# dmlc/dgl

Hardware: AMD Instinct MI355X
Metric: edges/sec for g-SpMM copy_u+sum (feat=100); % HBM roofline (higher is better)
Workload: dtype f32; 1 GPU; configs[1]: g-SpMM copy_u+sum on ogbn-products-shaped CSR (N=2449029 rows, E=61859140 edges, feat=100) fp32, int32 ids, variant U; parallelism=1 GPU, tuning_flags=25

## Files before the change

dgl_amd/csrc/spmm_csr.hip.h:

```cpp
#pragma once
#include <algorithm>
#include <cstdlib>
#include <type_traits>

#include "common.h"

namespace dgla {

template <typename Idx>
struct SpmmParams {
  const Idx* indptr;
  const Idx* indices;
  const Idx* eids;
  int64_t num_rows, nnz, num_waves;
  int wave_items;
  const int64_t* plan;
  const void* ufeat;
  const void* efeat;
  void* out;
  Idx* arg_u;
  Idx* arg_e;
  int out_len, lhs_len, rhs_len;
  int log2_lpe;
  int rhs_group;
  BcastDims bd;
  int accumulate;
  int rhs_neg, rhs_div;
  int rhs_mask;
  int stage_w;
  int red_min;
  int arg_empty;
  int mean;
  uint32_t tune;
  const void* umain;
  const void* utail;
  const unsigned* split_meta;
  int split_main, split_tail;
  int split_edge_lines;
  int split_t16;
  int split_base16;
  int split_straddle_slack;
  int split_row_bytes, split_base_bytes;
  const uint8_t* rel;
  const void* const* xtab;
  const void* const* wtab;
  int num_rel;
  int wave_slots;
  unsigned* fix_count;
  int64_t* carry_row;
  void* carry_val;
  void* tail_val;
  Idx* carry_argu;
  Idx* carry_arge;
  Idx* tail_argu;
  Idx* tail_arge;
};

template <typename Idx>
__global__ void spmm_merge_plan_kernel(const Idx* __restrict__ indptr, int64_t num_rows,
                                       int64_t nnz, int64_t num_waves,
                                       int64_t* __restrict__ plan, int wave_items) {
  const int64_t w = blockIdx.x * static_cast<int64_t>(blockDim.x) + threadIdx.x;
  if (w > num_waves) return;
  int64_t d = w * wave_items;
  const int64_t total = num_rows + nnz;
  if (d > total) d = total;
  int64_t lo = 0, hi = num_rows;
  while (lo < hi) {
    const int64_t mid = (lo + hi + 1) >> 1;
    if (static_cast<int64_t>(indptr[mid]) + mid <= d)
      lo = mid;
    else
      hi = mid - 1;
  }
  plan[w] = lo;
}

template <typename DT, int VEC>
__device__ __forceinline__ void store_nt(DT* dst, const VecT<DT, VEC>& v) {
  constexpr int B = sizeof(DT) * VEC;
  if constexpr (B == 16) {
// ... 168 lines not shown
}
template <typename T>
__device__ __forceinline__ void st_sc1(T* p, T v) {
  __hip_atomic_store((__attribute__((address_space(1))) T*)p, v, __ATOMIC_RELAXED, __HIP_MEMORY_SCOPE_AGENT);
}

template <typename DT>
__device__ __forceinline__ bool mask_bit(DT w, int k) {
  if constexpr (sizeof(DT) == 2) {
    uint16_t b;
    __builtin_memcpy(&b, &w, 2);
    return (b >> (k & 15)) & 1;
  } else if constexpr (sizeof(DT) == 4) {
    uint32_t b;
    __builtin_memcpy(&b, &w, 4);
    return (b >> (k & 31)) & 1;
  } else {
    uint64_t b;
    __builtin_memcpy(&b, &w, 8);
    return (b >> (k & 63)) & 1;
  }
}

template <typename Idx, typename DT, int VEC, int OP, int RED, int BC, int U, bool MULTI = false,
          bool NTR = false>
__global__ __launch_bounds__(64 * kWavesPerBlock) void spmm_csr_merge_kernel(
    const SpmmParams<Idx> p) {
  using A = typename Acc<DT>::type;
  constexpr bool UL = op_uses_lhs(OP), UR = op_uses_rhs(OP);
  constexpr bool ARG = RED != kSum;
  constexpr bool TU = UL && !MULTI, TE = UR || MULTI;
  constexpr int RV = (BC == kBcNone) ? VEC : 1;

  __shared__ int s_cols[UL ? kWavesPerBlock : 1][UL ? kWaveItems : 1];
  __shared__ int s_rend[kWavesPerBlock][kWaveItems + 2];
  extern __shared__ __align__(8) unsigned char s_dyn[];
  __shared__ uint8_t s_rel[MULTI ? kWavesPerBlock : 1][MULTI ? kWaveItems : 1];
  __shared__ const DT* s_tx[(MULTI && UL) ? 256 : 1];
  __shared__ const DT* s_tw[(MULTI && UR) ? 256 : 1];
  if constexpr (MULTI) {
    for (int i = threadIdx.x; i < p.num_rel; i += 64 * kWavesPerBlock) {
      if constexpr (UL) s_tx[i] = static_cast<const DT*>(p.xtab[i]);
      if constexpr (UR) s_tw[i] = static_cast<const DT*>(p.wtab[i]);
    }
  }

  const int wib = threadIdx.x >> 6;
  const int lane = threadIdx.x & 63;
  unsigned blk = blockIdx.x;
  if ((p.tune & kTuneXcd) && gridDim.y == 1) {
    const unsigned nb = gridDim.x, q = nb >> 3, r = nb & 7u;
    const unsigned x = blk & 7u, i = blk >> 3;
    blk = x * q + (x < r ? x : r) + i;
  }
  const int64_t w = static_cast<int64_t>(blk) * kWavesPerBlock + wib;
  const bool has_eid = p.eids != nullptr;
  constexpr bool kStageW = UL && UR && !MULTI && !NTR && BC == kBcRhsGroup && RED == kSum && sizeof(DT) == 4;
  [[maybe_unused]] const bool stage_w = kStageW && p.stage_w != 0;

  int64_t i0 = 0, j0 = 0;
  int R = 0, nE = 0;
  if (w < p.num_waves) {
    const int64_t total = p.num_rows + p.nnz;
    const int64_t d0 = w * p.wave_items;
    int64_t d1 = d0 + p.wave_items;
    if (d1 > total) d1 = total;
    i0 = p.plan[w];
    const int64_t i1 = p.plan[w + 1];
    j0 = d0 - i0;
    R = static_cast<int>(i1 - i0);
    nE = static_cast<int>((d1 - i1) - j0);
    const int items = nE + R;
    if (items > 0) {
      Idx itemv[kWaveItems / 64];
      Idx eidv[kWaveItems / 64];
      [[maybe_unused]] uint32_t wv[kStageW ? kWaveItems / 64 : 1];
      uint8_t relv[MULTI ? kWaveItems / 64 : 1];
#pragma unroll
      for (int k = 0; k < kWaveItems / 64; ++k) {
        if (64 * k >= p.wave_items) break;
        int it = lane + 64 * k;
        if (it >= items) it = items - 1;
        const Idx* src = p.indptr + (i0 + 1 + (it < nE ? 0 : it - nE));
        if constexpr (UL) src = it < nE ? p.indices + (j0 + it) : src;
        itemv[k] = *src;
        if constexpr (MULTI) relv[k] = it < nE ? p.rel[j0 + it] : uint8_t(0);
        if constexpr (UR) {
          if (has_eid) {
            const int ie = it < nE ? it : (nE > 0 ? nE - 1 : 0);
            eidv[k] = nE > 0 ? load_global<Idx, 1>(p.eids + (j0 + ie)).v[0] : static_cast<Idx>(p.arg_empty);
          }
          if constexpr (kStageW) {
            if (stage_w && !has_eid)
              wv[k] = nE > 0 ? load_global<uint32_t, 1>(static_cast<const uint32_t*>(p.efeat) + (j0 + (it < nE ? it : nE - 1))).v[0] : 0u;
          }
        }
      }
      if constexpr (kStageW) {
        if (stage_w && has_eid) {
#pragma unroll
          for (int k = 0; k < kWaveItems / 64; ++k) {
            if (64 * k >= p.wave_items) break;
            wv[k] = nE > 0 ? load_global<uint32_t, 1>(static_cast<const uint32_t*>(p.efeat) + static_cast<int64_t>(eidv[k])).v[0] : 0u;
          }
        }
      }
      const int64_t first = static_cast<int64_t>(p.indptr[i0]) - j0;
#pragma unroll
      for (int k = 0; k < kWaveItems / 64; ++k) {
        if (64 * k >= p.wave_items) break;
        const int it = lane + 64 * k;
        if (it < nE) {
          if constexpr (UL) s_cols[wib][it] = static_cast<int>(itemv[k]);
          if constexpr (UR) {
            bool staged = false;
            if constexpr (kStageW) {
              if (stage_w) {
                reinterpret_cast<uint32_t*>(s_dyn)[wib * kWaveItems + it] = wv[k];
                staged = true;
              }
            }
            if (!staged && has_eid) reinterpret_cast<Idx*>(s_dyn)[wib * kWaveItems + it] = eidv[k];
          }
          if constexpr (MULTI) s_rel[wib][it] = relv[k];
        } else if (it < items) {
          s_rend[wib][it - nE + 1] = static_cast<int>(static_cast<int64_t>(itemv[k]) - j0);
        }
      }
      if (lane == 0) s_rend[wib][0] = first < 0 ? -1 : static_cast<int>(first);
    } else if (lane == 0) {
      s_rend[wib][0] = 0;
    }
  }
  __syncthreads();
  if (w >= p.num_waves) return;

  const int lpe = 1 << p.log2_lpe;
  const int g = lane >> p.log2_lpe;
  const int lg = lane & (lpe - 1);
  const int G = 64 >> p.log2_lpe;
  const int Tg = p.wave_items >> (6 - p.log2_lpe);
  const int F = p.out_len;
  const int k0 = (static_cast<int>(blockIdx.y) * 64 + lg) * VEC;
  if (k0 >= F) return;

  typedef const __attribute__((address_space(3))) int* lds_int_ptr;
  typedef const __attribute__((address_space(3))) Idx* lds_idx_ptr;
  const lds_int_ptr cols = (lds_int_ptr)s_cols[UL ? wib : 0];
  const lds_int_ptr rend = (lds_int_ptr)s_rend[wib];
  const lds_idx_ptr eidl = (lds_idx_ptr)s_dyn + wib * kWaveItems;

  const int items = R + nE;
  int dlo = g * Tg, dhi = dlo + Tg;
  if (dlo > items) dlo = items;
  if (dhi > items) dhi = items;
  auto rows_before = [&](int d) {
    int lo = 0, hi = R;
    while (lo < hi) {
      const int mid = (lo + hi) >> 1;
      if (rend[mid + 1] + mid < d)
        lo = mid + 1;
      else
        hi = mid;
    }
    return lo;
  };
  const int t_s = rows_before(dlo), t_e = rows_before(dhi);
  const int e_s = dlo - t_s, e_e = dhi - t_e;
  const bool wslots = (RED == kSum) && p.wave_slots != 0;
  const int64_t slot = wslots ? w : w * G + g;

  int lo_off = k0, ro_off = k0;
  if constexpr (BC == kBcRhsGroup) ro_off = k0 / p.rhs_group;
  if constexpr (BC == kBcGeneral) bcast_offsets(p.bd, k0, &lo_off, &ro_off);
  const DT* __restrict__ X = static_cast<const DT*>(p.ufeat) + lo_off;
  const DT* __restrict__ Wt = static_cast<const DT*>(p.efeat) + ro_off;
  const int64_t lhs_len = p.lhs_len;
  const int64_t rhs_len = p.rhs_len;
  constexpr int E16 = 16 / static_cast<int>(sizeof(DT));
  bool edge_layout = false;
  [[maybe_unused]] unsigned ej = 0u;
  [[maybe_unused]] int e_piece_lo = 0, e_piece_hi = 0;
  [[maybe_unused]] int e_pitch = 0;
  [[maybe_unused]] const DT* e_side = nullptr;
  bool straddle = false;
  if (p.split_main > 0 && p.split_straddle_slack >= 0) {
    if constexpr (UL && !MULTI && VEC * sizeof(DT) == 8) straddle = split_wanted(p.split_meta);
  } else if (p.split_main > 0 && p.split_edge_lines > 0 && split_wanted(p.split_meta)) {
    {
      if constexpr (UL && !MULTI && VEC * sizeof(DT) == 16) {
        edge_layout = true;
        const int j = lo_off / E16, rp = p.lhs_len / E16;
        if (j >= rp - p.split_t16) {
          ej = 0x40000000u;
          e_side = static_cast<const DT*>(p.utail);
          e_pitch = p.split_t16 * E16;
          e_piece_lo = e_piece_hi = (j - (rp - p.split_t16)) * E16;
        } else {
          ej = static_cast<unsigned>(j);
          e_side = static_cast<const DT*>(p.umain);
          e_pitch = 8 * E16;
// ... 96 lines not shown
            const unsigned head = 8u - o16;
            const bool in_place = (ej - head) < e_in_place;
            const int side_off = ej < head ? e_piece_lo : e_piece_hi;
            const DT* base = in_place ? X : e_side;
            const int64_t pitch = in_place ? lhs_len : static_cast<int64_t>(e_pitch);
            const int add = in_place ? 0 : side_off;
            ptr = reinterpret_cast<const XV*>(base + (c * pitch + add));
            done = true;
          }
        }
        if constexpr (VEC * sizeof(DT) == 8) {
          if (straddle) {
            const unsigned o = static_cast<unsigned>((static_cast<uint64_t>(c) * static_cast<unsigned>(p.split_row_bytes) +
                                                      static_cast<unsigned>(p.split_base_bytes)) & 127u);
            const bool from_side = o > static_cast<unsigned>(p.split_straddle_slack);
            const DT* base = from_side ? static_cast<const DT*>(p.umain) + lo_off : X;
            const int64_t pitch = from_side ? static_cast<int64_t>(p.split_main) : lhs_len;
            ptr = reinterpret_cast<const XV*>(base + c * pitch);
            done = true;
          }
        }
        if (!done) ptr = reinterpret_cast<const XV*>(X + c * lhs_len);
        uint64_t wb = 0;
        __builtin_memcpy(&wb, &b.w[u].v[0], sizeof(DT));
        const bool wanted = ((wb >> (k0 & (BITS - 1))) & ((1u << VEC) - 1u)) != 0u;
        b.x[u] = *(wanted ? ptr : gate_dummy);
      }
    }
  };

  [[maybe_unused]] auto load_batch_sw = [&](int e, Batch& b) {
    if constexpr (kStageW) {
      typedef const __attribute__((address_space(3))) uint32_t* lds_u32_ptr;
      const lds_u32_ptr sw = (lds_u32_ptr)s_dyn + wib * kWaveItems;
#pragma unroll
      for (int u = 0; u < U; ++u) {
        int ee = e + u;
        if (ee >= e_e) ee = e_e - 1;
        const int64_t c = cols[ee];
        bool done = false;
        if constexpr (VEC * sizeof(DT) == 16) {
          if (edge_layout) {
            const unsigned o16 = (e_t16 * static_cast<unsigned>(c) + e_base16) & 7u;
            const unsigned head = 8u - o16;
            const bool in_place = (ej - head) < e_in_place;
            const int side_off = ej < head ? e_piece_lo : e_piece_hi;
            const DT* base = in_place ? X : e_side;
            const int64_t pitch = in_place ? lhs_len : static_cast<int64_t>(e_pitch);
            const int add = in_place ? 0 : side_off;
            b.x[u] = *reinterpret_cast<const XV*>(base + (c * pitch + add));
            done = true;
          }
        }
        if constexpr (VEC * sizeof(DT) == 8) {
          if (straddle) {
            const unsigned o = static_cast<unsigned>((static_cast<uint64_t>(c) * static_cast<unsigned>(p.split_row_bytes) +
                                                      static_cast<unsigned>(p.split_base_bytes)) & 127u);
            const bool from_side = o > static_cast<unsigned>(p.split_straddle_slack);
            const DT* base = from_side ? static_cast<const DT*>(p.umain) + lo_off : X;
            const int64_t pitch = from_side ? static_cast<int64_t>(p.split_main) : lhs_len;
            b.x[u] = *reinterpret_cast<const XV*>(base + c * pitch);
            done = true;
          }
        }
        if (!done) b.x[u] = *reinterpret_cast<const XV*>(X + c * lhs_len);
        const uint32_t wbits = sw[ee];
        __builtin_memcpy(&b.w[u].v[0], &wbits, 4);
// ... 19 lines not shown
  auto edge_name = [&](int bi) -> Idx {
    if (bi < 0) return static_cast<Idx>(p.arg_empty);
    if constexpr (MULTI)
      return static_cast<Idx>(j0 + bi);
    else if constexpr (UR)
      return has_eid ? eidl[bi] : static_cast<Idx>(j0 + bi);
    else
      return Idx(0);
  };
  DT* __restrict__ out = static_cast<DT*>(p.out);
  bool first_is_tail = rend[t_s] < e_s;
  [[maybe_unused]] A treg[VEC];
  [[maybe_unused]] bool have_tail = false;
  [[maybe_unused]] int tail_t = 0;

  const bool fuse = p.fix_count != nullptr;
  [[maybe_unused]] int64_t tail_pending = -1;
  auto put_part = [&](A* dst, const A (&vals)[VEC]) {
    if (fuse) {
#pragma unroll
      for (int v = 0; v < VEC; ++v) st_sc1(dst + v, vals[v]);
    } else {
#pragma unroll
      for (int v = 0; v < VEC; ++v) dst[v] = vals[v];
    }
  };
  auto put_arg = [&](Idx* dst, Idx val) {
    if (fuse)
      st_sc1(dst, val);
    else
      *dst = val;
  };

  auto flush = [&](int t) {
    const int64_t row = i0 + t;
    if (first_is_tail && RED == kSum && wslots && g == 1) {
#pragma unroll
      for (int v = 0; v < VEC; ++v) treg[v] = acc[v];
      have_tail = true;
      tail_t = t;
      first_is_tail = false;
    } else if (first_is_tail) {
      put_part(static_cast<A*>(p.tail_val) + slot * F + k0, acc);
      if constexpr (ARG) {
#pragma unroll
        for (int v = 0; v < VEC; ++v) {
          const int bi = best[v];
          if constexpr (TU) put_arg(p.tail_argu + slot * F + k0 + v, bi >= 0 ? static_cast<Idx>(cols[bi]) : static_cast<Idx>(p.arg_empty));
          if constexpr (TE) put_arg(p.tail_arge + slot * F + k0 + v, edge_name(bi));
        }
      }
      tail_pending = row;
      first_is_tail = false;
    } else {
      DT* o = out + row * F + k0;
      VecT<DT, VEC> ov;
      if (p.accumulate) {
        ov = *reinterpret_cast<VecT<DT, VEC>*>(o);
#pragma unroll
        for (int v = 0; v < VEC; ++v) ov.v[v] = from_acc<DT>(to_acc<DT>(ov.v[v]) + acc[v]);
      } else if (RED == kSum && p.mean) {
        const A den = round_to_storage<DT>(static_cast<A>(cnt > 1 ? cnt : 1));
#pragma unroll
        for (int v = 0; v < VEC; ++v) ov.v[v] = from_acc<DT>(round_to_storage<DT>(acc[v]) / den);
      } else {
#pragma unroll
        for (int v = 0; v < VEC; ++v) ov.v[v] = from_acc<DT>(acc[v]);
      }
// ... 55 lines not shown
            if constexpr (TE) ae[v] = geti(pe + base + v);
          }
        }
      }
    };
    for (int64_t q = s_first + 1; q < s_last; ++q) combine(cv, p.carry_argu, p.carry_arge, q * F + k0);
    combine(tv, p.tail_argu, p.tail_arge, s_last * F + k0);
    DT* o = out + R * F + k0;
    VecT<DT, VEC> ov;
    if (RED == kSum && p.mean) {
      const int64_t deg = rb - ra;
      const A den = round_to_storage<DT>(static_cast<A>(deg > 1 ? deg : 1));
#pragma unroll
      for (int v = 0; v < VEC; ++v) ov.v[v] = from_acc<DT>(round_to_storage<DT>(tot[v]) / den);
    } else if (p.accumulate) {
      ov = *reinterpret_cast<VecT<DT, VEC>*>(o);
#pragma unroll
      for (int v = 0; v < VEC; ++v) ov.v[v] = from_acc<DT>(to_acc<DT>(ov.v[v]) + tot[v]);
    } else {
#pragma unroll
      for (int v = 0; v < VEC; ++v) ov.v[v] = from_acc<DT>(tot[v]);
    }
    *reinterpret_cast<VecT<DT, VEC>*>(o) = ov;
    if constexpr (ARG) {
#pragma unroll
      for (int v = 0; v < VEC; ++v) {
        if constexpr (TU) p.arg_u[R * F + k0 + v] = au[v];
        if constexpr (TE) p.arg_e[R * F + k0 + v] = ae[v];
      }
    }
  };

  int t = t_s;
  int next_end = (t < R) ? rend[t + 1] : 0x7fffffff;
  [[maybe_unused]] const bool rhs_neg = p.rhs_neg != 0, rhs_div = p.rhs_div != 0, rhs_mask = p.rhs_mask != 0;

  auto reduce_batch = [&](int e, const Batch& b) {
#pragma unroll
    for (int u = 0; u < U; ++u) {
      const int ee = e + u;
      if (ee < e_e) {
        while (ee >= next_end) {
          flush(t);
          ++t;
          next_end = (t < R) ? rend[t + 1] : 0x7fffffff;
        }
#pragma unroll
        for (int v = 0; v < VEC; ++v) {
          A l = A(0), r = A(0);
          if constexpr (UL) l = to_acc<DT>(b.x[u].v[v]);
          if constexpr (UR) r = to_acc<DT>(b.w[u].v[RV == 1 ? 0 : v]);
          A raw;
          if constexpr (OP == kAdd)
            raw = l + (rhs_neg ? -r : r);
          else if constexpr (OP == kMul && BC == kBcRhsGroup)
            raw = rhs_mask ? (mask_bit<DT>(b.w[u].v[0], k0 + v) ? l : A(0)) : (rhs_div ? l / r : l * r);
          else if constexpr (OP == kMul)
            raw = rhs_div ? l / r : l * r;
          else
            raw = apply_op<OP, A>(l, r);
          const A val = round_to_storage<DT>(raw);
          if constexpr (RED == kSum) {
            acc[v] += val;
          } else {
            if (red_min ? acc[v] > val : acc[v] < val) {
              acc[v] = val;
              best[v] = ee;
            }
          }
        }
        ++cnt;
      }
    }
  };

  bool gated_done = false;
  if constexpr (kGated) {
    if (rhs_mask && VEC <= static_cast<int>(8 * sizeof(DT)) && (p.tune & kTuneNoGate) == 0) {
// ... 19 lines not shown
    }
  }
  if constexpr (kStageW) {
    if (stage_w && !gated_done) {
      gated_done = true;
      if (e_s < e_e) {
        int e = e_s;
        Batch ba, bb;
        load_batch_sw(e, ba);
        for (; e < e_e; e += 2 * U) {
          load_batch_sw(e + U, bb);
          reduce_batch(e, ba);
          load_batch_sw(e + 2 * U, ba);
          reduce_batch(e + U, bb);
        }
      }
    }
  }
  if (!gated_done && e_s < e_e) {
    int e = e_s;
    Batch ba, bb;
    load_batch(e, ba);
    for (; e < e_e; e += 2 * U) {
      load_batch(e + U, bb);
      reduce_batch(e, ba);
      load_batch(e + 2 * U, ba);
      reduce_batch(e + U, bb);
    }
  }
  while (t < t_e) {
    flush(t);
    ++t;
  }

  if constexpr (RED == kSum) {
    if (wslots) {
      A c0[VEC];
#pragma unroll
      for (int v = 0; v < VEC; ++v) c0[v] = __shfl_xor(acc[v], 32, 64);
      const int cnt0 = __shfl_xor(cnt, 32, 64);
      if (g == 1) {
        const bool g0_carry = cnt0 > 0;
        int64_t crow = -1;
        if (have_tail) {
          A tot[VEC];
#pragma unroll
          for (int v = 0; v < VEC; ++v) tot[v] = c0[v] + treg[v];
          const bool began_here = tail_t > 0 || rend[0] >= 0;
          if (began_here) {
            DT* o = out + (i0 + tail_t) * F + k0;
            VecT<DT, VEC> ov;
            if (p.accumulate) {
              ov = *reinterpret_cast<VecT<DT, VEC>*>(o);
#pragma unroll
              for (int v = 0; v < VEC; ++v) ov.v[v] = from_acc<DT>(to_acc<DT>(ov.v[v]) + tot[v]);
            } else if (p.mean) {
              const int deg = rend[tail_t + 1] - rend[tail_t];
              const A den = round_to_storage<DT>(static_cast<A>(deg > 1 ? deg : 1));
#pragma unroll
              for (int v = 0; v < VEC; ++v) ov.v[v] = from_acc<DT>(round_to_storage<DT>(tot[v]) / den);
            } else {
#pragma unroll
              for (int v = 0; v < VEC; ++v) ov.v[v] = from_acc<DT>(tot[v]);
            }
            *reinterpret_cast<VecT<DT, VEC>*>(o) = ov;
          } else {
            put_part(static_cast<A*>(p.tail_val) + slot * F + k0, tot);
            tail_pending = i0 + tail_t;
          }
          if (cnt > 0) {
            crow = i0 + t;
            put_part(static_cast<A*>(p.carry_val) + slot * F + k0, acc);
          }
        } else if (g0_carry || cnt > 0) {
          crow = i0 + t;
          A cvv[VEC];
#pragma unroll
          for (int v = 0; v < VEC; ++v) cvv[v] = g0_carry ? (cnt > 0 ? c0[v] + acc[v] : c0[v]) : acc[v];
          put_part(static_cast<A*>(p.carry_val) + slot * F + k0, cvv);
        }
        if (!fuse && lg == 0) p.carry_row[slot] = crow;
        if (fuse && crow >= 0) finish_run(crow);
      }
      if (fuse && tail_pending >= 0) finish_run(tail_pending);
      return;
    }
  }
  const bool has_carry = cnt > 0;
  if (!fuse && lg == 0 && blockIdx.y == 0) p.carry_row[slot] = has_carry ? i0 + t : int64_t(-1);
  if (has_carry) {
    put_part(static_cast<A*>(p.carry_val) + slot * F + k0, acc);
    if constexpr (ARG) {
#pragma unroll
      for (int v = 0; v < VEC; ++v) {
        const int bi = best[v];
        if constexpr (TU) put_arg(p.carry_argu + slot * F + k0 + v, bi >= 0 ? static_cast<Idx>(cols[bi]) : static_cast<Idx>(p.arg_empty));
        if constexpr (TE) put_arg(p.carry_arge + slot * F + k0 + v, edge_name(bi));
      }
    }
  }
  if (fuse) {
    if (tail_pending >= 0) finish_run(tail_pending);
    if (has_carry) finish_run(i0 + t);
  }
}

template <typename Idx, typename DT, int OP, int RED, bool MULTI = false>
__global__ __launch_bounds__(64) void spmm_csr_fixup_kernel(const SpmmParams<Idx> p,
                                                            int64_t num_slots) {
  using A = typename Acc<DT>::type;
  constexpr bool UL = op_uses_lhs(OP) && !MULTI, UR = op_uses_rhs(OP) || MULTI;
  constexpr bool ARG = RED != kSum;
  for (int64_t s = blockIdx.x; s < num_slots; s += gridDim.x) {
    const int64_t row = p.carry_row[s];
    if (row < 0) continue;
    if (s > 0 && p.carry_row[s - 1] == row) continue;
    int64_t s2 = s + 1;
    for (;;) {
      const int64_t q = s2 + threadIdx.x;
      const bool same = q < num_slots && p.carry_row[q] == row;
      const uint64_t m = __ballot(same);
      if (m != ~uint64_t(0)) {
        s2 += __builtin_ctzll(~m);
        break;
      }
      s2 += 64;
    }
    const int F = p.out_len;
    const A* cv = static_cast<const A*>(p.carry_val);
    const A* tv = static_cast<const A*>(p.tail_val);
    DT* out = static_cast<DT*>(p.out);
    for (int k = threadIdx.x; k < F; k += 64) {
      A acc = cv[s * F + k];
      Idx au = 0, ae = 0;
      if constexpr (ARG) {
        if constexpr (UL) au = p.carry_argu[s * F + k];
        if constexpr (UR) ae = p.carry_arge[s * F + k];
      }
      auto combine = [&](A val, Idx cu, Idx ce) {
        if constexpr (RED == kSum) {
          acc += val;
        } else {
          const bool take = p.red_min ? (acc > val) : (acc < val);
          if (take) {
            acc = val;
            if constexpr (UL) au = cu;
            if constexpr (UR) ae = ce;
          }
        }
      };
      const A tval = tv[s2 * F + k];
      Idx tu = 0, te = 0;
      if constexpr (ARG) {
        if constexpr (UL) tu = p.tail_argu[s2 * F + k];
        if constexpr (UR) te = p.tail_arge[s2 * F + k];
      }
      int64_t q = s + 1;
      for (; q + 8 <= s2; q += 8) {
        A v[8];
        Idx vu[8], ve[8];
#pragma unroll
        for (int u = 0; u < 8; ++u) {
          v[u] = cv[(q + u) * F + k];
          vu[u] = ve[u] = 0;
          if constexpr (ARG) {
            if constexpr (UL) vu[u] = p.carry_argu[(q + u) * F + k];
            if constexpr (UR) ve[u] = p.carry_arge[(q + u) * F + k];
          }
        }
#pragma unroll
        for (int u = 0; u < 8; ++u) combine(v[u], vu[u], ve[u]);
      }
      for (; q < s2; ++q) {
        Idx cu = 0, ce = 0;
        if constexpr (ARG) {
          if constexpr (UL) cu = p.carry_argu[q * F + k];
          if constexpr (UR) ce = p.carry_arge[q * F + k];
        }
        combine(cv[q * F + k], cu, ce);
      }
      combine(tval, tu, te);
      const int64_t o = row * F + k;
      if (RED == kSum && p.mean) {
        const int64_t deg = static_cast<int64_t>(p.indptr[row + 1]) - static_cast<int64_t>(p.indptr[row]);
        acc = round_to_storage<DT>(acc) / round_to_storage<DT>(static_cast<A>(deg > 1 ? deg : 1));
      }
      if (p.accumulate)
        out[o] = from_acc<DT>(to_acc<DT>(out[o]) + acc);
      else
        out[o] = from_acc<DT>(acc);
      if constexpr (ARG) {
        if constexpr (UL) p.arg_u[o] = au;
        if constexpr (UR) p.arg_e[o] = ae;
      }
    }
  }
}

constexpr int kFuseMaxGroups = 8;

constexpr int64_t kFuseMaxWaves = 32768;
inline bool spmm_fuse_fixup_enabled(int64_t num_waves, int64_t rows, int64_t nnz) {
  const char* e = getenv("DGLA_SPMM_FUSE_FIXUP");
  if (e && (e[0] == '0' || e[0] == '1')) return e[0] == '1';
  return num_waves < kFuseMaxWaves && nnz < 64 * rows;
}

struct SpmmGeometry {
  int vec;
  int log2_lpe;
  int groups;
  int chunks;
  int wave_slots;
  int wave_items;
  int64_t num_waves, num_slots;
  size_t off_plan, off_meta, off_fixcnt, off_carry_row, off_carry_val, off_tail_val, off_carry_argu,
      off_carry_arge, off_tail_argu, off_tail_arge, total;
  int split_main_bytes, split_tail_bytes;
  size_t off_split_main, off_split_tail;
  int split_edge_lines;
  bool split_straddle;
};

constexpr int64_t kSplitProbeWindowRows = 65536;

constexpr int64_t kSmallGraphUnits = 4096;

inline int64_t spmm_split_min_bytes() {
  const char* e = getenv("DGLA_SPLIT_MIN_MB");
  const int64_t mb = e && atoll(e) > 0 ? atoll(e) : 16;
  return mb << 20;
}

inline bool spmm_split_shape_ok(const SpmmLaunch& L, size_t elem_bytes) {
  if (!(L.tune & kTuneSplit) || L.rel != nullptr || !op_uses_lhs(L.op)) return false;
  if (L.bcast == kBcGeneral || L.lhs_len != L.out_len) return false;
  const int64_t rb = L.lhs_len * static_cast<int64_t>(elem_bytes);
  if (rb % 8 || rb > 1024 || rb < 128 || rb % 128 == 0) return false;
// ... 141 lines not shown
  p.umain = p.utail = nullptr;
  p.split_meta = nullptr;
  p.split_main = p.split_tail = 0;
  p.split_edge_lines = p.split_t16 = p.split_base16 = 0;
  p.split_straddle_slack = -1;
  p.split_row_bytes = p.split_base_bytes = 0;
  if (g.split_straddle) {
    p.umain = ws + g.off_split_main;
    if (!(L.tune & kTuneSplitForce) && !L.split_keep)
      p.split_meta = reinterpret_cast<const unsigned*>(ws + g.off_meta);
    p.split_main = g.split_main_bytes / static_cast<int>(sizeof(DT));
    p.split_row_bytes = static_cast<int>(L.lhs_len * static_cast<int64_t>(sizeof(DT)));
    p.split_straddle_slack = g.split_main_bytes - p.split_row_bytes;
    p.split_base_bytes = static_cast<int>(reinterpret_cast<uintptr_t>(L.ufeat) & 127u);
  } else if (g.split_main_bytes > 0) {
    p.umain = ws + g.off_split_main;
    p.utail = ws + g.off_split_tail;
    if (!(L.tune & kTuneSplitForce) && !L.split_keep)
      p.split_meta = reinterpret_cast<const unsigned*>(ws + g.off_meta);
    p.split_main = g.split_main_bytes / static_cast<int>(sizeof(DT));
    p.split_tail = g.split_tail_bytes / static_cast<int>(sizeof(DT));
    p.split_edge_lines = g.split_edge_lines;
    p.split_t16 = g.split_tail_bytes / 16;
    p.split_base16 = static_cast<int>((reinterpret_cast<uintptr_t>(L.ufeat) & 127u) >> 4);
  }
  p.rel = static_cast<const uint8_t*>(L.rel);
  p.xtab = L.ufeat_tab;
  p.wtab = L.efeat_tab;
  p.num_rel = L.num_rel;
  p.wave_slots = g.wave_slots;
  p.fix_count = (g.chunks == 1 && (g.wave_slots || g.groups <= kFuseMaxGroups) && spmm_fuse_fixup_enabled(g.num_waves, L.csr.num_rows, L.csr.nnz))
                    ? reinterpret_cast<unsigned*>(ws + g.off_fixcnt)
                    : nullptr;
  p.carry_row = reinterpret_cast<int64_t*>(ws + g.off_carry_row);
  p.carry_val = ws + g.off_carry_val;
  p.tail_val = ws + g.off_tail_val;
  p.carry_argu = reinterpret_cast<Idx*>(ws + g.off_carry_argu);
  p.carry_arge = reinterpret_cast<Idx*>(ws + g.off_carry_arge);
  p.tail_argu = reinterpret_cast<Idx*>(ws + g.off_tail_argu);
  p.tail_arge = reinterpret_cast<Idx*>(ws + g.off_tail_arge);
  return p;
}

constexpr int kSpmmUnroll = 4;

inline bool spmm_nt_stream(const SpmmLaunch& L) {
  return L.csr.eids == nullptr && L.csr.nnz >= 64 * L.csr.num_rows;
}

template <typename Idx, typename DT, int VEC, int OP, int RED, int BC>
inline int launch_spmm_one(const SpmmLaunch& L, const SpmmGeometry& g) {
  SpmmParams<Idx> p = make_params<Idx, DT>(L, g);
  const unsigned blocks =
      static_cast<unsigned>((g.num_waves + kWavesPerBlock - 1) / kWavesPerBlock);
  if (g.split_straddle && !L.split_valid) {
    char* ws = static_cast<char*>(L.workspace);
    const int row_pieces = p.split_row_bytes / 8;
    const int64_t total = L.csr.num_cols * row_pieces;
    const unsigned sblocks = static_cast<unsigned>(std::min<int64_t>((total + 255) / 256, int64_t(1) << 20));
    hipLaunchKernelGGL(spmm_straddle_rows_kernel<0>, dim3(sblocks), dim3(256), 0, L.stream,
                       static_cast<const piece8_t*>(L.ufeat), reinterpret_cast<piece8_t*>(ws + g.off_split_main),
                       L.csr.num_cols, row_pieces, g.split_main_bytes / 8, p.split_straddle_slack,
                       static_cast<unsigned>(p.split_base_bytes), p.split_meta);
    DGLA_CHECK_HIP(hipGetLastError());
  } else if (g.split_edge_lines > 0 && !L.split_valid) {
    char* ws = static_cast<char*>(L.workspace);
    const int t16 = g.split_tail_bytes / 16, side = 8 + t16;
    const int row_pieces = static_cast<int>(L.lhs_len * static_cast<int64_t>(sizeof(DT)) / 16);
    const int64_t total = L.csr.num_cols * side;
    constexpr int K = 4;
    const unsigned sblocks =
        static_cast<unsigned>(std::min<int64_t>((total + 256 * K - 1) / (256 * K), int64_t(1) << 20));
    const unsigned magic = 0xFFFFFFFFu / static_cast<unsigned>(side) + 1u;
    hipLaunchKernelGGL(spmm_split_edges_kernel<K>, dim3(sblocks), dim3(256), 0, L.stream,
                       static_cast<const piece16_t*>(L.ufeat),
                       reinterpret_cast<piece16_t*>(ws + g.off_split_main),
                       reinterpret_cast<piece16_t*>(ws + g.off_split_tail), L.csr.num_cols, row_pieces,
                       t16, 8 * g.split_edge_lines, magic, p.split_meta,
                       static_cast<unsigned>(p.split_base16));
    DGLA_CHECK_HIP(hipGetLastError());
  }
  if (L.prepare_only) return 0;
  unsigned dyn_lds = (op_uses_rhs(OP) && L.csr.eids != nullptr)
                         ? static_cast<unsigned>(kWavesPerBlock * kWaveItems * sizeof(Idx))
                         : 0u;
  if constexpr (op_uses_lhs(OP) && op_uses_rhs(OP) && BC == kBcRhsGroup && RED == kSum && sizeof(DT) == 4) {
    if (L.rel == nullptr && L.rhs_len == 1 && !L.rhs_mask && L.efeat != nullptr && (L.tune & kTuneNoStageW) == 0) {
      p.stage_w = 1;
      dyn_lds = std::max<unsigned>(dyn_lds, static_cast<unsigned>(kWavesPerBlock * kWaveItems * sizeof(uint32_t)));
    }
  }
  const ProfileEvents pe = profile_events();
  if (pe.before) DGLA_CHECK_HIP(hipEventRecord(pe.before, L.stream));
  if (L.rel != nullptr) {
    if constexpr ((OP == kCopyLhs || OP == kCopyRhs || OP == kMul) && BC != kBcGeneral) {
      if (L.op == kDiv) {
        last_error() = "stacked SpMM supports copy_lhs / copy_rhs / mul only";
        return -1;
      }
      hipLaunchKernelGGL((spmm_csr_merge_kernel<Idx, DT, VEC, OP, RED, BC, kSpmmUnroll, true>),
                         dim3(blocks, g.chunks), dim3(64 * kWavesPerBlock), dyn_lds, L.stream, p);
      if constexpr (RED != kSum) {
        DGLA_CHECK_HIP(hipGetLastError());
        if (pe.after) DGLA_CHECK_HIP(hipEventRecord(pe.after, L.stream));
        if (p.fix_count) return 0;
        hipLaunchKernelGGL((spmm_csr_fixup_kernel<Idx, DT, OP, RED, true>),
                           dim3(static_cast<unsigned>(std::min<int64_t>(g.num_slots, int64_t(1) << 24))),
                           dim3(64), 0, L.stream, p, g.num_slots);
        DGLA_CHECK_HIP(hipGetLastError());
        return 0;
      }
    } else {
      last_error() = "stacked SpMM supports copy_lhs / copy_rhs / mul only";
      return -1;
    }
  } else if (OP == kCopyRhs && BC == kBcNone && !L.accumulate && spmm_nt_stream(L)) {
    if constexpr (OP == kCopyRhs && BC == kBcNone)
      hipLaunchKernelGGL((spmm_csr_merge_kernel<Idx, DT, VEC, OP, RED, BC, kSpmmUnroll, false, true>),
                         dim3(blocks, g.chunks), dim3(64 * kWavesPerBlock), dyn_lds, L.stream, p);
  } else {
    hipLaunchKernelGGL((spmm_csr_merge_kernel<Idx, DT, VEC, OP, RED, BC, kSpmmUnroll, false>),
                       dim3(blocks, g.chunks), dim3(64 * kWavesPerBlock), dyn_lds, L.stream, p);
  }
  DGLA_CHECK_HIP(hipGetLastError());
  if (pe.after) DGLA_CHECK_HIP(hipEventRecord(pe.after, L.stream));
  if (p.fix_count) return 0;
  hipLaunchKernelGGL((spmm_csr_fixup_kernel<Idx, DT, OP, RED>),
                     dim3(static_cast<unsigned>(std::min<int64_t>(g.num_slots, int64_t(1) << 24))),
                     dim3(64), 0, L.stream, p, g.num_slots);
  DGLA_CHECK_HIP(hipGetLastError());
  return 0;
}

template <typename Idx, typename DT, int VEC, int OP, int RED>
inline int launch_spmm_bc(const SpmmLaunch& L, const SpmmGeometry& g) {
  if constexpr (!op_uses_rhs(OP) || OP == kCopyRhs) {
    return launch_spmm_one<Idx, DT, VEC, OP, RED, kBcNone>(L, g);
  } else {
    switch (L.bcast) {
      case kBcNone: return launch_spmm_one<Idx, DT, VEC, OP, RED, kBcNone>(L, g);
      case kBcRhsGroup: return launch_spmm_one<Idx, DT, VEC, OP, RED, kBcRhsGroup>(L, g);
      default:
        if constexpr (VEC == 1) return launch_spmm_one<Idx, DT, 1, OP, RED, kBcGeneral>(L, g);
    }
    last_error() = "internal: general broadcast needs the scalar path";
    return -1;
  }
}

template <typename Idx, typename DT, int VEC, int OP>
inline int launch_spmm_red(const SpmmLaunch& L, const SpmmGeometry& g) {
  switch (L.red) {
    case kSum: return launch_spmm_bc<Idx, DT, VEC, OP, kSum>(L, g);
    case kMax:
    case kMin: return launch_spmm_bc<Idx, DT, VEC, OP, kMax>(L, g);
  }
  last_error() = "unsupported SpMM reducer";
  return -1;
}

template <typename Idx, typename DT, int VEC>
inline int launch_spmm_op(const SpmmLaunch& L, const SpmmGeometry& g) {
// ... 90 lines not shown
```

Before: 13.58 billion edges/s.

## Let waves own short straddling rows and batch fixup slots per wave

When a merge-path wave ends inside a short row, the wave now loads that row's remaining edges (up to 64) into an extended LDS area. Its last lane group finishes the row and writes the output directly, and the next wave skips the prefix it would otherwise have emitted as a carry. This cuts the carry/tail partial writes and the work left for the fixup kernel. The fixup kernel is also restructured to use 4-wave blocks, with each wave scanning 8 slots via ballot instead of one block per slot. The cost is more per-wave LDS, extra indptr and index loads, and more branching.

```diff
diff --git a/dgl_amd/csrc/spmm_csr.hip.h b/dgl_amd/csrc/spmm_csr.hip.h
--- a/dgl_amd/csrc/spmm_csr.hip.h
+++ b/dgl_amd/csrc/spmm_csr.hip.h
@@ -6,6 +6,9 @@
 #include "common.h"
 
 namespace dgla {
+
+constexpr int kOwnMax = 64;
+constexpr int kUnitLds = kWaveItems + kOwnMax;
 
 template <typename Idx>
 struct SpmmParams {
@@ -47,6 +50,7 @@
   int num_rel;
   int wave_slots;
   unsigned* fix_count;
+  int own_rows;
   int64_t* carry_row;
   void* carry_val;
   void* tail_val;
@@ -281,7 +285,7 @@
   constexpr bool TU = UL && !MULTI, TE = UR || MULTI;
   constexpr int RV = (BC == kBcNone) ? VEC : 1;
 
-  __shared__ int s_cols[UL ? kWavesPerBlock : 1][UL ? kWaveItems : 1];
+  __shared__ int s_cols[UL ? kWavesPerBlock : 1][UL ? kUnitLds : 1];
   __shared__ int s_rend[kWavesPerBlock][kWaveItems + 2];
   extern __shared__ __align__(8) unsigned char s_dyn[];
   __shared__ uint8_t s_rel[MULTI ? kWavesPerBlock : 1][MULTI ? kWaveItems : 1];
@@ -306,6 +310,12 @@
   const bool has_eid = p.eids != nullptr;
   constexpr bool kStageW = UL && UR && !MULTI && !NTR && BC == kBcRhsGroup && RED == kSum && sizeof(DT) == 4;
   [[maybe_unused]] const bool stage_w = kStageW && p.stage_w != 0;
+
+  constexpr bool kOwn = RED == kSum && !MULTI;
+  const bool own_on = kOwn && p.own_rows != 0;
+  [[maybe_unused]] bool own_out = false;
+  [[maybe_unused]] int own_m = 0;
+  [[maybe_unused]] bool own_in_pre = false;
 
   int64_t i0 = 0, j0 = 0;
   int R = 0, nE = 0;
@@ -345,6 +355,25 @@
           }
         }
       }
+      [[maybe_unused]] Idx own_colv = 0, own_eidv = 0;
+      [[maybe_unused]] uint32_t own_wv = 0u;
+      [[maybe_unused]] int64_t own_a = 0, own_b = 0;
+      const bool own_try = own_on && nE > 0 && i1 < p.num_rows && d1 - d0 == p.wave_items;
+      if constexpr (kOwn) {
+        if (own_try) {
+          own_a = static_cast<int64_t>(p.indptr[i1]);
+          own_b = static_cast<int64_t>(p.indptr[i1 + 1]);
+          int64_t pos = j0 + nE + lane;
+          if (pos >= p.nnz) pos = p.nnz - 1;
+          if constexpr (UL) own_colv = p.indices[pos];
+          if constexpr (UR) {
+            if (has_eid) own_eidv = load_global<Idx, 1>(p.eids + pos).v[0];
+            if constexpr (kStageW) {
+              if (stage_w && !has_eid) own_wv = load_global<uint32_t, 1>(static_cast<const uint32_t*>(p.efeat) + pos).v[0];
+            }
+          }
+        }
+      }
       if constexpr (kStageW) {
         if (stage_w && has_eid) {
 #pragma unroll
@@ -352,9 +381,37 @@
             if (64 * k >= p.wave_items) break;
             wv[k] = nE > 0 ? load_global<uint32_t, 1>(static_cast<const uint32_t*>(p.efeat) + static_cast<int64_t>(eidv[k])).v[0] : 0u;
           }
-        }
-      }
+          if (own_try) own_wv = load_global<uint32_t, 1>(static_cast<const uint32_t*>(p.efeat) + static_cast<int64_t>(own_eidv)).v[0];
+        }
+      }
+      const int own_tg = p.wave_items >> (6 - p.log2_lpe);
+      const int own_slot_off = p.wave_slots != 0 ? 0 : p.wave_items - own_tg;
+      if constexpr (kOwn) {
+        if (own_try) {
+          const int64_t pos0 = own_a + i1;
+          const int64_t m = own_b - (j0 + nE);
+          own_out = pos0 >= d0 + own_slot_off && pos0 < d1 && m + 1 <= std::min(kOwnMax, own_tg);
+          if (own_out) {
+            own_m = static_cast<int>(m);
+            if (lane < own_m) {
+              if constexpr (UL) s_cols[wib][nE + lane] = static_cast<int>(own_colv);
+              if constexpr (UR) {
+                bool staged = false;
+                if constexpr (kStageW) {
+                  if (stage_w) {
+                    reinterpret_cast<uint32_t*>(s_dyn)[wib * kUnitLds + nE + lane] = own_wv;
+                    staged = true;
+                  }
+                }
+                if (!staged && has_eid) reinterpret_cast<Idx*>(s_dyn)[wib * kUnitLds + nE + lane] = own_eidv;
+              }
+            }
+          }
+        }
+      }
+      if (lane == 0) s_rend[wib][R + 1] = own_out ? nE : 0x7fffffff;
       const int64_t first = static_cast<int64_t>(p.indptr[i0]) - j0;
+      own_in_pre = own_on && first < 0 && first >= static_cast<int64_t>(own_slot_off) - p.wave_items;
 #pragma unroll
       for (int k = 0; k < kWaveItems / 64; ++k) {
         if (64 * k >= p.wave_items) break;
@@ -365,11 +422,11 @@
             bool staged = false;
             if constexpr (kStageW) {
               if (stage_w) {
-                reinterpret_cast<uint32_t*>(s_dyn)[wib * kWaveItems + it] = wv[k];
+                reinterpret_cast<uint32_t*>(s_dyn)[wib * kUnitLds + it] = wv[k];
                 staged = true;
               }
             }
-            if (!staged && has_eid) reinterpret_cast<Idx*>(s_dyn)[wib * kWaveItems + it] = eidv[k];
+            if (!staged && has_eid) reinterpret_cast<Idx*>(s_dyn)[wib * kUnitLds + it] = eidv[k];
           }
           if constexpr (MULTI) s_rel[wib][it] = relv[k];
         } else if (it < items) {
@@ -379,6 +436,7 @@
       if (lane == 0) s_rend[wib][0] = first < 0 ? -1 : static_cast<int>(first);
     } else if (lane == 0) {
       s_rend[wib][0] = 0;
+      s_rend[wib][1] = 0x7fffffff;
     }
   }
   __syncthreads();
@@ -397,7 +455,7 @@
   typedef const __attribute__((address_space(3))) Idx* lds_idx_ptr;
   const lds_int_ptr cols = (lds_int_ptr)s_cols[UL ? wib : 0];
   const lds_int_ptr rend = (lds_int_ptr)s_rend[wib];
-  const lds_idx_ptr eidl = (lds_idx_ptr)s_dyn + wib * kWaveItems;
+  const lds_idx_ptr eidl = (lds_idx_ptr)s_dyn + wib * kUnitLds;
 
   const int items = R + nE;
   int dlo = g * Tg, dhi = dlo + Tg;
@@ -414,8 +472,21 @@
     }
     return lo;
   };
-  const int t_s = rows_before(dlo), t_e = rows_before(dhi);
-  const int e_s = dlo - t_s, e_e = dhi - t_e;
+  int t_s = rows_before(dlo), t_e = rows_before(dhi);
+  int e_s = dlo - t_s, e_e = dhi - t_e;
+  [[maybe_unused]] bool own_here = false;
+  if constexpr (kOwn) {
+    const bool own_in = own_in_pre && R >= 1 && rend[1] + 1 <= std::min(kOwnMax, Tg);
+    if (own_in && g == 0) {
+      t_s = 1;
+      e_s = rend[1];
+    }
+    own_here = own_out && g == G - 1;
+    if (own_here) {
+      e_e = nE + own_m;
+      t_e = R + 1;
+    }
+  }
   const bool wslots = (RED == kSum) && p.wave_slots != 0;
   const int64_t slot = wslots ? w : w * G + g;
 
@@ -578,7 +649,7 @@
   [[maybe_unused]] auto load_batch_sw = [&](int e, Batch& b) {
     if constexpr (kStageW) {
       typedef const __attribute__((address_space(3))) uint32_t* lds_u32_ptr;
-      const lds_u32_ptr sw = (lds_u32_ptr)s_dyn + wib * kWaveItems;
+      const lds_u32_ptr sw = (lds_u32_ptr)s_dyn + wib * kUnitLds;
 #pragma unroll
       for (int u = 0; u < U; ++u) {
         int ee = e + u;
@@ -664,8 +735,18 @@
       *dst = val;
   };
 
+  __shared__ A s_own[kOwn ? kWavesPerBlock : 1][kOwn ? 64 * VEC : 1];
+
   auto flush = [&](int t) {
     const int64_t row = i0 + t;
+    if constexpr (kOwn) {
+      if (own_here && t == R) {
+#pragma unroll
+        for (int v = 0; v < VEC; ++v) s_own[wib][lane * VEC + v] = acc[v];
+        reset();
+        return;
+      }
+    }
     if (first_is_tail && RED == kSum && wslots && g == 1) {
 #pragma unroll
       for (int v = 0; v < VEC; ++v) treg[v] = acc[v];
@@ -787,7 +868,7 @@
   };
 
   int t = t_s;
-  int next_end = (t < R) ? rend[t + 1] : 0x7fffffff;
+  int next_end = (t <= R) ? rend[t + 1] : 0x7fffffff;
   [[maybe_unused]] const bool rhs_neg = p.rhs_neg != 0, rhs_div = p.rhs_div != 0, rhs_mask = p.rhs_mask != 0;
 
   auto reduce_batch = [&](int e, const Batch& b) {
@@ -798,7 +879,7 @@
         while (ee >= next_end) {
           flush(t);
           ++t;
-          next_end = (t < R) ? rend[t + 1] : 0x7fffffff;
+          next_end = (t <= R) ? rend[t + 1] : 0x7fffffff;
         }
 #pragma unroll
         for (int v = 0; v < VEC; ++v) {
@@ -884,6 +965,37 @@
     flush(t);
     ++t;
   }
+  [[maybe_unused]] A own_c[kOwn ? VEC : 1];
+  if constexpr (kOwn) {
+    if (own_here) {
+#pragma unroll
+      for (int v = 0; v < VEC; ++v) {
+        own_c[v] = acc[v];
+        acc[v] = s_own[wib][lane * VEC + v];
+      }
+      cnt = 1;
+    }
+  }
+  [[maybe_unused]] auto own_finish = [&](const A (&carry)[VEC]) {
+    if constexpr (kOwn) {
+      DT* o = out + (i0 + R) * F + k0;
+      VecT<DT, VEC> ov;
+      if (p.mean) {
+        const int64_t deg = static_cast<int64_t>(p.indptr[i0 + R + 1]) - static_cast<int64_t>(p.indptr[i0 + R]);
+        const A den = round_to_storage<DT>(static_cast<A>(deg > 1 ? deg : 1));
+#pragma unroll
+        for (int v = 0; v < VEC; ++v) ov.v[v] = from_acc<DT>(round_to_storage<DT>(carry[v] + own_c[v]) / den);
+      } else if (p.accumulate) {
+        ov = *reinterpret_cast<VecT<DT, VEC>*>(o);
+#pragma unroll
+        for (int v = 0; v < VEC; ++v) ov.v[v] = from_acc<DT>(to_acc<DT>(ov.v[v]) + (carry[v] + own_c[v]));
+      } else {
+#pragma unroll
+        for (int v = 0; v < VEC; ++v) ov.v[v] = from_acc<DT>(carry[v] + own_c[v]);
+      }
+      *reinterpret_cast<VecT<DT, VEC>*>(o) = ov;
+    }
+  };
 
   if constexpr (RED == kSum) {
     if (wslots) {
@@ -920,16 +1032,22 @@
             put_part(static_cast<A*>(p.tail_val) + slot * F + k0, tot);
             tail_pending = i0 + tail_t;
           }
-          if (cnt > 0) {
+          if (own_here) {
+            own_finish(acc);
+          } else if (cnt > 0) {
             crow = i0 + t;
             put_part(static_cast<A*>(p.carry_val) + slot * F + k0, acc);
           }
         } else if (g0_carry || cnt > 0) {
-          crow = i0 + t;
           A cvv[VEC];
 #pragma unroll
           for (int v = 0; v < VEC; ++v) cvv[v] = g0_carry ? (cnt > 0 ? c0[v] + acc[v] : c0[v]) : acc[v];
-          put_part(static_cast<A*>(p.carry_val) + slot * F + k0, cvv);
+          if (own_here) {
+            own_finish(cvv);
+          } else {
+            crow = i0 + t;
+            put_part(static_cast<A*>(p.carry_val) + slot * F + k0, cvv);
+          }
         }
         if (!fuse && lg == 0) p.carry_row[slot] = crow;
         if (fuse && crow >= 0) finish_run(crow);
@@ -938,7 +1056,13 @@
       return;
     }
   }
-  const bool has_carry = cnt > 0;
+  bool has_carry = cnt > 0;
+  if constexpr (kOwn) {
+    if (own_here) {
+      own_finish(acc);
+      has_carry = false;
+    }
+  }
   if (!fuse && lg == 0 && blockIdx.y == 0) p.carry_row[slot] = has_carry ? i0 + t : int64_t(-1);
   if (has_carry) {
     put_part(static_cast<A*>(p.carry_val) + slot * F + k0, acc);
@@ -957,93 +1081,113 @@
   }
 }
 
+constexpr int kFixSlotsPerWave = 8;
+constexpr int kFixWavesPerBlock = 4;
+inline unsigned spmm_fixup_blocks(int64_t num_slots) {
+  const int64_t per_block = kFixSlotsPerWave * kFixWavesPerBlock;
+  return static_cast<unsigned>(std::max<int64_t>(1, std::min<int64_t>((num_slots + per_block - 1) / per_block, int64_t(1) << 22)));
+}
+
 template <typename Idx, typename DT, int OP, int RED, bool MULTI = false>
-__global__ __launch_bounds__(64) void spmm_csr_fixup_kernel(const SpmmParams<Idx> p,
-                                                            int64_t num_slots) {
+__global__ __launch_bounds__(64 * kFixWavesPerBlock) void spmm_csr_fixup_kernel(const SpmmParams<Idx> p,
+                                                                                 int64_t num_slots) {
   using A = typename Acc<DT>::type;
   constexpr bool UL = op_uses_lhs(OP) && !MULTI, UR = op_uses_rhs(OP) || MULTI;
   constexpr bool ARG = RED != kSum;
-  for (int64_t s = blockIdx.x; s < num_slots; s += gridDim.x) {
-    const int64_t row = p.carry_row[s];
-    if (row < 0) continue;
-    if (s > 0 && p.carry_row[s - 1] == row) continue;
-    int64_t s2 = s + 1;
-    for (;;) {
-      const int64_t q = s2 + threadIdx.x;
-      const bool same = q < num_slots && p.carry_row[q] == row;
-      const uint64_t m = __ballot(same);
-      if (m != ~uint64_t(0)) {
-        s2 += __builtin_ctzll(~m);
-        break;
-      }
-      s2 += 64;
-    }
-    const int F = p.out_len;
-    const A* cv = static_cast<const A*>(p.carry_val);
-    const A* tv = static_cast<const A*>(p.tail_val);
-    DT* out = static_cast<DT*>(p.out);
-    for (int k = threadIdx.x; k < F; k += 64) {
-      A acc = cv[s * F + k];
-      Idx au = 0, ae = 0;
-      if constexpr (ARG) {
-        if constexpr (UL) au = p.carry_argu[s * F + k];
-        if constexpr (UR) ae = p.carry_arge[s * F + k];
-      }
-      auto combine = [&](A val, Idx cu, Idx ce) {
-        if constexpr (RED == kSum) {
-          acc += val;
-        } else {
-          const bool take = p.red_min ? (acc > val) : (acc < val);
-          if (take) {
-            acc = val;
-            if constexpr (UL) au = cu;
-            if constexpr (UR) ae = ce;
-          }
-        }
-      };
-      const A tval = tv[s2 * F + k];
-      Idx tu = 0, te = 0;
-      if constexpr (ARG) {
-        if constexpr (UL) tu = p.tail_argu[s2 * F + k];
-        if constexpr (UR) te = p.tail_arge[s2 * F + k];
-      }
-      int64_t q = s + 1;
-      for (; q + 8 <= s2; q += 8) {
-        A v[8];
-        Idx vu[8], ve[8];
-#pragma unroll
-        for (int u = 0; u < 8; ++u) {
-          v[u] = cv[(q + u) * F + k];
-          vu[u] = ve[u] = 0;
+  const int lane = threadIdx.x & 63;
+  const int64_t wave = static_cast<int64_t>(blockIdx.x) * kFixWavesPerBlock + (threadIdx.x >> 6);
+  const int64_t wave_stride = static_cast<int64_t>(gridDim.x) * kFixWavesPerBlock * kFixSlotsPerWave;
+  for (int64_t base = wave * kFixSlotsPerWave; base < num_slots; base += wave_stride) {
+    int64_t my_row = -1;
+    bool lead = false;
+    if (lane < kFixSlotsPerWave && base + lane < num_slots) {
+      my_row = p.carry_row[base + lane];
+      lead = my_row >= 0 && (base + lane == 0 || p.carry_row[base + lane - 1] != my_row);
+    }
+    uint64_t live = __ballot(lead);
+    while (live != 0) {
+      const int li = __builtin_ctzll(live);
+      live &= live - 1;
+      const int64_t s = base + li;
+      const int64_t row = __shfl(my_row, li, 64);
+      int64_t s2 = s + 1;
+      for (;;) {
+        const int64_t q = s2 + lane;
+        const bool same = q < num_slots && p.carry_row[q] == row;
+        const uint64_t m = __ballot(same);
+        if (m != ~uint64_t(0)) {
+          s2 += __builtin_ctzll(~m);
+          break;
+        }
+        s2 += 64;
+      }
+      const int F = p.out_len;
+      const A* cv = static_cast<const A*>(p.carry_val);
+      const A* tv = static_cast<const A*>(p.tail_val);
+      DT* out = static_cast<DT*>(p.out);
+      for (int k = lane; k < F; k += 64) {
+        A acc = cv[s * F + k];
+        Idx au = 0, ae = 0;
+        if constexpr (ARG) {
+          if constexpr (UL) au = p.carry_argu[s * F + k];
+          if constexpr (UR) ae = p.carry_arge[s * F + k];
+        }
+        auto combine = [&](A val, Idx cu, Idx ce) {
+          if constexpr (RED == kSum) {
+            acc += val;
+          } else {
+            const bool take = p.red_min ? (acc > val) : (acc < val);
+            if (take) {
+              acc = val;
+              if constexpr (UL) au = cu;
+              if constexpr (UR) ae = ce;
+            }
+          }
+        };
+        const A tval = tv[s2 * F + k];
+        Idx tu = 0, te = 0;
+        if constexpr (ARG) {
+          if constexpr (UL) tu = p.tail_argu[s2 * F + k];
+          if constexpr (UR) te = p.tail_arge[s2 * F + k];
+        }
+        int64_t q = s + 1;
+        for (; q + 8 <= s2; q += 8) {
+          A v[8];
+          Idx vu[8], ve[8];
+#pragma unroll
+          for (int u = 0; u < 8; ++u) {
+            v[u] = cv[(q + u) * F + k];
+            vu[u] = ve[u] = 0;
+            if constexpr (ARG) {
+              if constexpr (UL) vu[u] = p.carry_argu[(q + u) * F + k];
+              if constexpr (UR) ve[u] = p.carry_arge[(q + u) * F + k];
+            }
+          }
+#pragma unroll
+          for (int u = 0; u < 8; ++u) combine(v[u], vu[u], ve[u]);
+        }
+        for (; q < s2; ++q) {
+          Idx cu = 0, ce = 0;
           if constexpr (ARG) {
-            if constexpr (UL) vu[u] = p.carry_argu[(q + u) * F + k];
-            if constexpr (UR) ve[u] = p.carry_arge[(q + u) * F + k];
-          }
-        }
-#pragma unroll
-        for (int u = 0; u < 8; ++u) combine(v[u], vu[u], ve[u]);
-      }
-      for (; q < s2; ++q) {
-        Idx cu = 0, ce = 0;
+            if constexpr (UL) cu = p.carry_argu[q * F + k];
+            if constexpr (UR) ce = p.carry_arge[q * F + k];
+          }
+          combine(cv[q * F + k], cu, ce);
+        }
+        combine(tval, tu, te);
+        const int64_t o = row * F + k;
+        if (RED == kSum && p.mean) {
+          const int64_t deg = static_cast<int64_t>(p.indptr[row + 1]) - static_cast<int64_t>(p.indptr[row]);
+          acc = round_to_storage<DT>(acc) / round_to_storage<DT>(static_cast<A>(deg > 1 ? deg : 1));
+        }
+        if (p.accumulate)
+          out[o] = from_acc<DT>(to_acc<DT>(out[o]) + acc);
+        else
+          out[o] = from_acc<DT>(acc);
         if constexpr (ARG) {
-          if constexpr (UL) cu = p.carry_argu[q * F + k];
-          if constexpr (UR) ce = p.carry_arge[q * F + k];
-        }
-        combine(cv[q * F + k], cu, ce);
-      }
-      combine(tval, tu, te);
-      const int64_t o = row * F + k;
-      if (RED == kSum && p.mean) {
-        const int64_t deg = static_cast<int64_t>(p.indptr[row + 1]) - static_cast<int64_t>(p.indptr[row]);
-        acc = round_to_storage<DT>(acc) / round_to_storage<DT>(static_cast<A>(deg > 1 ? deg : 1));
-      }
-      if (p.accumulate)
-        out[o] = from_acc<DT>(to_acc<DT>(out[o]) + acc);
-      else
-        out[o] = from_acc<DT>(acc);
-      if constexpr (ARG) {
-        if constexpr (UL) p.arg_u[o] = au;
-        if constexpr (UR) p.arg_e[o] = ae;
+          if constexpr (UL) p.arg_u[o] = au;
+          if constexpr (UR) p.arg_e[o] = ae;
+        }
       }
     }
   }
@@ -1056,6 +1200,11 @@
   const char* e = getenv("DGLA_SPMM_FUSE_FIXUP");
   if (e && (e[0] == '0' || e[0] == '1')) return e[0] == '1';
   return num_waves < kFuseMaxWaves && nnz < 64 * rows;
+}
+
+inline bool spmm_own_rows_enabled() {
+  const char* e = getenv("DGLA_SPMM_OWN_ROWS");
+  return !(e && e[0] == '0');
 }
 
 struct SpmmGeometry {
@@ -1263,6 +1412,7 @@
   p.fix_count = (g.chunks == 1 && (g.wave_slots || g.groups <= kFuseMaxGroups) && spmm_fuse_fixup_enabled(g.num_waves, L.csr.num_rows, L.csr.nnz))
                     ? reinterpret_cast<unsigned*>(ws + g.off_fixcnt)
                     : nullptr;
+  p.own_rows = (g.chunks == 1 && L.rel == nullptr && L.red == kSum && spmm_own_rows_enabled()) ? 1 : 0;
   p.carry_row = reinterpret_cast<int64_t*>(ws + g.off_carry_row);
   p.carry_val = ws + g.off_carry_val;
   p.tail_val = ws + g.off_tail_val;
@@ -1313,12 +1463,12 @@
   }
   if (L.prepare_only) return 0;
   unsigned dyn_lds = (op_uses_rhs(OP) && L.csr.eids != nullptr)
-                         ? static_cast<unsigned>(kWavesPerBlock * kWaveItems * sizeof(Idx))
+                         ? static_cast<unsigned>(kWavesPerBlock * kUnitLds * sizeof(Idx))
                          : 0u;
   if constexpr (op_uses_lhs(OP) && op_uses_rhs(OP) && BC == kBcRhsGroup && RED == kSum && sizeof(DT) == 4) {
     if (L.rel == nullptr && L.rhs_len == 1 && !L.rhs_mask && L.efeat != nullptr && (L.tune & kTuneNoStageW) == 0) {
       p.stage_w = 1;
-      dyn_lds = std::max<unsigned>(dyn_lds, static_cast<unsigned>(kWavesPerBlock * kWaveItems * sizeof(uint32_t)));
+      dyn_lds = std::max<unsigned>(dyn_lds, static_cast<unsigned>(kWavesPerBlock * kUnitLds * sizeof(uint32_t)));
     }
   }
   const ProfileEvents pe = profile_events();
@@ -1335,9 +1485,8 @@
         DGLA_CHECK_HIP(hipGetLastError());
         if (pe.after) DGLA_CHECK_HIP(hipEventRecord(pe.after, L.stream));
         if (p.fix_count) return 0;
-        hipLaunchKernelGGL((spmm_csr_fixup_kernel<Idx, DT, OP, RED, true>),
-                           dim3(static_cast<unsigned>(std::min<int64_t>(g.num_slots, int64_t(1) << 24))),
-                           dim3(64), 0, L.stream, p, g.num_slots);
+        hipLaunchKernelGGL((spmm_csr_fixup_kernel<Idx, DT, OP, RED, true>), dim3(spmm_fixup_blocks(g.num_slots)),
+                           dim3(64 * kFixWavesPerBlock), 0, L.stream, p, g.num_slots);
         DGLA_CHECK_HIP(hipGetLastError());
         return 0;
       }
@@ -1356,9 +1505,8 @@
   DGLA_CHECK_HIP(hipGetLastError());
   if (pe.after) DGLA_CHECK_HIP(hipEventRecord(pe.after, L.stream));
   if (p.fix_count) return 0;
-  hipLaunchKernelGGL((spmm_csr_fixup_kernel<Idx, DT, OP, RED>),
-                     dim3(static_cast<unsigned>(std::min<int64_t>(g.num_slots, int64_t(1) << 24))),
-                     dim3(64), 0, L.stream, p, g.num_slots);
+  hipLaunchKernelGGL((spmm_csr_fixup_kernel<Idx, DT, OP, RED>), dim3(spmm_fixup_blocks(g.num_slots)),
+                     dim3(64 * kFixWavesPerBlock), 0, L.stream, p, g.num_slots);
   DGLA_CHECK_HIP(hipGetLastError());
   return 0;
 }
```

New measurement: 13.58 billion edges/s. About the same (-0.0%).
